# MasterBin-IIAU/Unicorn

Measured on AMD Instinct MI355X. Metric: frames/sec @ 800x1280 unicorn_track_large, higher is better.
Workload: dtype f16x2 (fp32-equivalent: split-f16 MFMA operands, fp32 accumulate); 1 GPU; unicorn_track_large SOT per-frame step 800x1280 (backbone+FPN, deform interaction, embedding, fp32-equivalent correlation, head); one independent stream per GPU, 16 consecutive frames per step; model=unicorn_track_large, task=sot, precision=f16x2, streams=1, distinct_frames_per_batch=16, weights=synthetic (oracle/synth.py), corr_dtype=f32-equivalent (f16x2 split operands, fp32 accumulate), accum=f32

## Files before the change

unicorn_amd/csrc/gemm_h2q.hip:

```cpp
#include "kernels.h"
#include "gemm_epi.h"


namespace {
constexpr int NW = 8;
constexpr int BM = 256, BN = 256, BKE = 32, ROWB = 128;
constexpr int HALF = 128 * ROWB;
constexpr int STAGE = 4 * HALF;
constexpr int OPER = 2 * STAGE;
constexpr int STG = 4096;
constexpr int LDS_BYTES = OPER + NW * STG;

struct Tile { int m0, n0, k0, split; };
struct ATile { __amdgpu_buffer_rsrc_t rs; int vo[2][2]; };
__device__ __forceinline__ Tile tile_of(int u, int nbm, int nbn, int nku) {
    const SplitTilePos t = supertile_split_pos(u, nbm, nbn, BM, BN);
    return {t.bm, t.bn, t.split * nku, t.split};
}
}

#define Q_WAIT_LDS() asm volatile("s_waitcnt lgkmcnt(0)" ::: "memory")

template <int ACT, bool OUTF, bool CONV, bool STATS, int FMT>
__global__ __launch_bounds__(64 * NW) void gemm_h2q_kernel(GemmArgs p) {
    constexpr int EB = FMT == FMT_H2 ? 4 : 2;
    constexpr int KS = ROWB / EB;
    extern __shared__ __attribute__((aligned(16))) char smem[];
    const int tid = threadIdx.x;
    const int lane = tid & 63;
    const int wave = __builtin_amdgcn_readfirstlane(tid >> 6);
    const int grp = wave >> 2, wc = wave & 3;
    const int fr = lane & 31, fh = lane >> 5;

    const int nbm = (p.M + BM - 1) / BM, nbn = (p.N + BN - 1) / BN;
    const int nunits = nbm * nbn * (p.splitk > 1 ? p.splitk : 1);
    int first, stride, count;
    persistent_units(blockIdx.x, gridDim.x, nunits, first, stride, count);
    if (count == 0) return;

    const int lrow = lane >> 3;
    const int lch = (lane & 7) ^ ((4 * (wave & 1) + (lrow >> 1)) & 7);
    const int lda4 = p.lda * EB, ldw4 = p.Kpad * EB;
    int vob[2][2];
#pragma unroll
    for (int h = 0; h < 2; ++h)
#pragma unroll
        for (int i = 0; i < 2; ++i) vob[h][i] = ((wave >> 2) * 64 + 8 * (wave & 3) + lrow + 128 * i + 32 * h) * ldw4 + lch * 16;
    const int arow = 8 * wave + lrow;
    auto make_a = [&](Tile tl, ATile& c) __attribute__((always_inline)) {
        char* abase = const_cast<char*>(reinterpret_cast<const char*>(p.A));
        if (!CONV) {
            const int rows = min(BM, p.M - tl.m0);
            c.rs = __builtin_amdgcn_make_buffer_rsrc(abase + (long)tl.m0 * lda4, 0, rows * lda4, 0x00020000);
#pragma unroll
            for (int h = 0; h < 2; ++h)
#pragma unroll
                for (int i = 0; i < 2; ++i) c.vo[h][i] = (arow + 128 * i + 64 * h) * lda4 + lch * 16;
        } else {
            const int b0 = tl.m0 / p.Mper, q0 = tl.m0 - b0 * p.Mper, oy0 = q0 / p.Wout, ox0 = q0 - oy0 * p.Wout;
            const int pix0 = (b0 * p.Hin + oy0 * p.stride) * p.Win + ox0 * p.stride;
            c.rs = __builtin_amdgcn_make_buffer_rsrc(abase + ((long)pix0 - (p.pad * p.Win + p.pad)) * lda4, 0, 0x7ffffff0, 0x00020000);
#pragma unroll
            for (int h = 0; h < 2; ++h)
#pragma unroll
                for (int i = 0; i < 2; ++i) {
                    const int m = tl.m0 + arow + 128 * i + 64 * h;
                    const bool ok = m < p.M;
                    const int mm = ok ? m : tl.m0;
                    const int b = mm / p.Mper, q = mm - b * p.Mper, oy = q / p.Wout, ox = q - oy * p.Wout;
                    const int off = ((b * p.Hin + oy * p.stride) * p.Win + ox * p.stride - pix0) * lda4 + lch * 16;
                    int bits = 0;
#pragma unroll
                    for (int t = 0; t < 3; ++t) {
                        const int iy = oy * p.stride - p.pad + t, ix = ox * p.stride - p.pad + t;
                        bits |= (t < p.KH && iy >= 0 && iy < p.Hin) ? (1 << t) : 0;
                        bits |= (t < p.KW && ix >= 0 && ix < p.Win) ? (8 << t) : 0;
                    }
                    c.vo[h][i] = off | ((ok ? bits : 0) << 26);
                }
        }
    };
    auto rsrc_b = [&](Tile tl) __attribute__((always_inline)) {
        return __builtin_amdgcn_make_buffer_rsrc(const_cast<char*>(reinterpret_cast<const char*>(p.W)) + (long)tl.n0 * ldw4, 0, BN * ldw4, 0x00020000);
    };
    const int cs = CONV ? p.Cin / KS : 1;
    const int csm = tap_csm(cs);
    const int kwm = tap_kwm(p.KW);
    auto issueA = [&](int h, int par, int kt, const ATile& c) __attribute__((always_inline)) {
        char* dst = smem + par * STAGE + h * HALF + wave * 1024;
        if (!CONV) {
            lds_dma16_buf(c.rs, dst, c.vo[h][0], kt * ROWB);
            lds_dma16_buf(c.rs, dst + 8192, c.vo[h][1], kt * ROWB);
        } else {
            const int tap = tap_index(kt, csm), cstep = kt - tap * cs;
            const int ky = tap_row(tap, kwm), kx = tap - ky * p.KW;
            const int soff = (ky * p.Win + kx) * lda4 + cstep * ROWB;
#pragma unroll
            for (int i = 0; i < 2; ++i) {
                const bool ok = ((c.vo[h][i] >> (26 + ky)) & (c.vo[h][i] >> (29 + kx)) & 1) != 0;
                lds_dma16_buf(c.rs, dst + i * 8192, ok ? (c.vo[h][i] & DESC_OFFSET_MASK) : DESC_OUT_OF_RANGE, soff);
            }
        }
    };
    auto issueB = [&](int h, int par, int kt, __amdgpu_buffer_rsrc_t rs) __attribute__((always_inline)) {
        char* dst = smem + par * STAGE + (2 + h) * HALF + wave * 1024;
        lds_dma16_buf(rs, dst, vob[h][0], kt * ROWB);
        lds_dma16_buf(rs, dst + 8192, vob[h][1], kt * ROWB);
    };

    const int sw = (fr >> 1) & 7;
    const int q0 = FMT == FMT_H2 ? 2 * fh : fh, q1 = FMT == FMT_H2 ? 2 * fh + 1 : 2 + fh;
    const int q2 = FMT == FMT_H2 ? 4 + 2 * fh : 4 + fh, q3 = FMT == FMT_H2 ? 5 + 2 * fh : 6 + fh;
    const int a_rd = (grp * 64 + fr) * ROWB, b_rd = 2 * HALF + (wc * 32 + fr) * ROWB;
    const int lds0 = (int)(size_t)(__attribute__((address_space(3))) char*)smem;
    if (lds0 != 0) __builtin_trap();
    int ra4[4] = {lds0 + a_rd + ((q0 ^ sw) << 4), lds0 + a_rd + ((q1 ^ sw) << 4), lds0 + a_rd + ((q2 ^ sw) << 4), lds0 + a_rd + ((q3 ^ sw) << 4)};
    int rb4[4] = {lds0 + b_rd + ((q0 ^ sw) << 4), lds0 + b_rd + ((q1 ^ sw) << 4), lds0 + b_rd + ((q2 ^ sw) << 4), lds0 + b_rd + ((q3 ^ sw) << 4)};

    f32x16 acc[4][2];
    f16x8 fa[2][4], fb[2][4];
    const int nk = (p.K / KS) / (p.splitk > 1 ? p.splitk : 1);
    Tile cur = tile_of(first, nbm, nbn, nk);
    Tile nxt = count > 1 ? tile_of(first + stride, nbm, nbn, nk) : cur;
    ATile ta_cur, ta_nxt;
    make_a(cur, ta_cur);
    make_a(nxt, ta_nxt);
    __amdgpu_buffer_rsrc_t rb_cur = rsrc_b(cur), rb_nxt = rsrc_b(nxt);

#define Q_LD_A(h)                                                                                   \
    _Pragma("unroll") for (int i = 0; i < 2; ++i) _Pragma("unroll") for (int q = 0; q < 4; ++q)      \
        fa[i][q] = lds_read_f16x8(ra4[q] + (h) * HALF + i * 32 * ROWB);
#define Q_LD_B(h) _Pragma("unroll") for (int q = 0; q < 4; ++q) fb[h][q] = lds_read_f16x8(rb4[q] + (h) * HALF);
#define Q_MF16(b, a, c) c = __builtin_amdgcn_mfma_f32_32x32x16_f16(b, a, c, 0, 0, 0)
#define Q_MB16(b, a, c) c = __builtin_amdgcn_mfma_f32_32x32x16_bf16(__builtin_bit_cast(bf16x8, b), __builtin_bit_cast(bf16x8, a), c, 0, 0, 0)
#define Q_MFMA(HA, HB)                                                                                   \
    if (FMT == FMT_H2) {                                                                                 \
        _Pragma("unroll") for (int kk = 0; kk < 2; ++kk) {                                               \
            Q_MF16(fb[HB][2 * kk + 1], fa[0][2 * kk], acc[2 * (HA)][HB]);                                \
            Q_MF16(fb[HB][2 * kk + 1], fa[1][2 * kk], acc[2 * (HA) + 1][HB]);                            \
            Q_MF16(fb[HB][2 * kk], fa[0][2 * kk + 1], acc[2 * (HA)][HB]);                                \
            Q_MF16(fb[HB][2 * kk], fa[1][2 * kk + 1], acc[2 * (HA) + 1][HB]);                            \
            Q_MF16(fb[HB][2 * kk], fa[0][2 * kk], acc[2 * (HA)][HB]);                                    \
            Q_MF16(fb[HB][2 * kk], fa[1][2 * kk], acc[2 * (HA) + 1][HB]);                                \
        }                                                                                                \
    } else {                                                                                             \
        _Pragma("unroll") for (int kk = 0; kk < 4; ++kk) {                                               \
            Q_MB16(fb[HB][kk], fa[0][kk], acc[2 * (HA)][HB]);                                            \
            Q_MB16(fb[HB][kk], fa[1][kk], acc[2 * (HA) + 1][HB]);                                        \
        }                                                                                                \
    }
#define Q_FUT(ahead)                                                   \
    int fk = kt + (ahead);                                             \
    const bool fnx = fk >= nk;                                         \
    fk -= fnx ? nk : 0;                                                \
    fk += fnx ? nxt.k0 : cur.k0;               \
    const __amdgpu_buffer_rsrc_t fb = fnx ? rb_nxt : rb_cur;                                  \
    ATile fa;                                                                                  \
    fa.rs = fnx ? ta_nxt.rs : ta_cur.rs;                                                       \
    _Pragma("unroll") for (int h_ = 0; h_ < 2; ++h_) _Pragma("unroll") for (int i_ = 0; i_ < 2; ++i_) {  \
        fa.vo[h_][i_] = (CONV && fnx) ? ta_nxt.vo[h_][i_] : ta_cur.vo[h_][i_];                 \
    }

    {
        const int kt = 0;
        issueA(0, 0, cur.k0, ta_cur); issueB(0, 0, cur.k0, rb_cur); issueB(1, 0, cur.k0, rb_cur); issueA(1, 0, cur.k0, ta_cur);
        Q_FUT(1);
        issueA(0, 1, fk, fa); issueB(1, 1, fk, fb); issueA(1, 1, fk, fa);
    }
    wait_vmcnt<6>();
    phase_barrier();
    if (grp == 1) phase_barrier();
    int par = 0;
#pragma unroll 1
    for (int t = 0; t < count; ++t) {
        ACC_CLEAR(acc, 4, 2);
#pragma unroll 1
        for (int kt = 0; kt < nk; ++kt) {
            {
                Q_LD_A(0); Q_LD_B(0);
                Q_WAIT_LDS();
                phase_barrier();
                if (!(p.dbg & 2)) { Q_MFMA(0, 0); }
                phase_barrier();
            }
            {
                Q_LD_B(1);
                if (!(p.dbg & 1)) { Q_FUT(1); issueB(0, par ^ 1, fk, fb); }
                if (!(p.dbg & 1)) { Q_FUT(2); issueA(0, par, fk, fa); }
                Q_WAIT_LDS();
                phase_barrier();
                if (!(p.dbg & 2)) { Q_MFMA(0, 1); }
                phase_barrier();
            }
            {
                Q_LD_A(1);
                Q_WAIT_LDS();
                phase_barrier();
                if (!(p.dbg & 2)) { Q_MFMA(1, 1); }
                phase_barrier();
            }
            {
                if (!(p.dbg & 1)) { Q_FUT(2); issueB(1, par, fk, fb); issueA(1, par, fk, fa); }
                wait_vmcnt<6>();
                Q_WAIT_LDS();
                phase_barrier();
                if (!(p.dbg & 2)) { Q_MFMA(1, 0); }
                phase_barrier();
            }
            par ^= 1;
#pragma unroll
            for (int q = 0; q < 4; ++q) { ra4[q] ^= STAGE; rb4[q] ^= STAGE; }
        }
        const Tile done = cur;
        cur = nxt; ta_cur = ta_nxt; rb_cur = rb_nxt;
        if (t + 2 < count) { nxt = tile_of(first + (t + 2) * stride, nbm, nbn, nk); make_a(nxt, ta_nxt); rb_nxt = rsrc_b(nxt); }
        char* st = smem + OPER + wave * STG;
        const int nw0 = done.n0 + wc * 64;
        const int rb0 = done.m0 + grp * 128;
        const int srow = p.splitk > 1 ? done.split * p.M : 0;
        if (p.dbg & 16) {
            float sacc = 0.f;
#pragma unroll
            for (int i = 0; i < 4; ++i)
#pragma unroll
                for (int j = 0; j < 2; ++j)
#pragma unroll
                    for (int r = 0; r < 16; ++r) sacc += acc[i][j][r];
            if (sacc == 1.2345e-30f && p.outF) p.outF[0] = sacc;
            continue;
        }
        if (STATS) {
            if (grp == 0) phase_barrier();
#pragma unroll
            for (int i = 0; i < 4; ++i)
#pragma unroll
                for (int j = 0; j < 2; ++j)
#pragma unroll
                    for (int r = 0; r < 16; ++r) acc[i][j][r] *= p.wscale;
        }
        const float ws = STATS ? 1.f : p.wscale;
        const bool has_res = OUTF && !STATS && !CONV && p.res != nullptr, has_b = p.outB != nullptr;
#pragma unroll
        for (int j = 0; j < 2; ++j) {
            float bv[16];
            {
                typedef float f32x8 __attribute__((ext_vector_type(8)));
                const __attribute__((address_space(4))) float* bias = (const __attribute__((address_space(4))) float*)(p.bias);
                if (!p.bias) {
#pragma unroll
                    for (int r = 0; r < 16; ++r) bv[r] = 0.f;
                } else if (nw0 + 64 <= p.N) {
#pragma unroll
                    for (int g = 0; g < 4; ++g) {
                        const f32x8 b8 = *reinterpret_cast<const __attribute__((address_space(4))) f32x8*>(bias + nw0 + j * 32 + 8 * g);
#pragma unroll
                        for (int e = 0; e < 4; ++e) bv[4 * g + e] = fh ? b8[4 + e] : b8[e];
                    }
                } else {
#pragma unroll
                    for (int g = 0; g < 4; ++g)
#pragma unroll
                        for (int e = 0; e < 4; ++e) {
                            const int c = nw0 + j * 32 + 8 * g + e;
                            const float lo = bias[min(c, p.N - 1)], hi = bias[min(c + 4, p.N - 1)];
                            bv[4 * g + e] = fh ? hi : lo;
                        }
                }
            }
#pragma unroll
            for (int i = 0; i < 4; ++i) {
                f32x4 rv[4];
                if (has_res) {
                    const int c = lane & 7, rr = lane >> 3;
                    const int col = nw0 + j * 32 + 4 * c;
#pragma unroll
                    for (int tt = 0; tt < 4; ++tt) {
                        const int row = rb0 + i * 32 + tt * 8 + rr;
                        const bool ok = row < p.M && col < p.N;
                        rv[tt] = *reinterpret_cast<const f32x4*>(p.res + (ok ? (size_t)row * p.ldr + col : 0));
                    }
                }
#pragma unroll
                for (int g = 0; g < 4; ++g) {
                    f32x4 v;
#pragma unroll
                    for (int e = 0; e < 4; ++e) v[e] = act_fast<ACT>(fmaf(acc[i][j][4 * g + e], ws, bv[4 * g + e]));
                    *reinterpret_cast<f32x4*>(st + fr * 128 + (((2 * g + fh) ^ (fr & 7)) << 4)) = v;
                }
                wave_lds_fence();
                if (OUTF) {
                    const int c = lane & 7, rr = lane >> 3;
                    const int col = nw0 + j * 32 + 4 * c;
#pragma unroll
                    for (int tt = 0; tt < 4; ++tt) {
                        const int r = tt * 8 + rr, row = rb0 + i * 32 + r;
                        f32x4 v = *reinterpret_cast<const f32x4*>(st + r * 128 + ((c ^ (r & 7)) << 4));
                        if (has_res) v += rv[tt];
                        if (row < p.M && col < p.N && !(p.dbg & 4)) {
                            const int orow = (p.out_hw ? (row / p.out_hw) * p.out_stride + p.out_off + row % p.out_hw : row) + srow;
                            *reinterpret_cast<f32x4*>(p.outF + (size_t)orow * p.ldf + col) = v;
                            if (has_b) act_store4(p.outB, (size_t)row * p.ldb + col, v[0], v[1], v[2], v[3], FMT);
                        }
                    }
                } else {
                    const int c = lane & 3, rr = lane >> 2;
                    const int col = nw0 + j * 32 + 8 * c;
#pragma unroll
                    for (int tt = 0; tt < 2; ++tt) {
                        const int r = tt * 16 + rr, row = rb0 + i * 32 + r;
                        const f32x4 lo = *reinterpret_cast<const f32x4*>(st + r * 128 + (((2 * c) ^ (r & 7)) << 4));
                        const f32x4 hi = *reinterpret_cast<const f32x4*>(st + r * 128 + (((2 * c + 1) ^ (r & 7)) << 4));
                        if (row < p.M && col < p.N && !(p.dbg & 4)) {
                            const float v8[8] = {lo[0], lo[1], lo[2], lo[3], hi[0], hi[1], hi[2], hi[3]};
                            if (FMT == FMT_H2) {
                                f16x8 h, l;
#pragma unroll
                                for (int q = 0; q < 8; ++q) { f16 hh, ll; h2_split(v8[q], hh, ll); h[q] = hh; l[q] = ll; }
                                char* op = reinterpret_cast<char*>(p.outB) + ((size_t)row * p.ldb + col) * 4;
                                __builtin_nontemporal_store(__builtin_bit_cast(f32x4, h), reinterpret_cast<f32x4*>(op));
                                __builtin_nontemporal_store(__builtin_bit_cast(f32x4, l), reinterpret_cast<f32x4*>(op + 16));
                            } else {
                                bf16x8 o;
#pragma unroll
                                for (int q = 0; q < 8; ++q) o[q] = (bf16)v8[q];
                                __builtin_nontemporal_store(__builtin_bit_cast(f32x4, o), reinterpret_cast<f32x4*>(p.outB + (size_t)row * p.ldb + col));
                            }
                        }
                    }
                }
                wave_lds_fence();
            }
        }
        if (STATS) {
            gemm_stats<2, 4, 4, 2>(p, acc, done.m0, done.n0, grp, wc, lane, tid, reinterpret_cast<float*>(smem + OPER));
            __syncthreads();
            if (grp == 1) phase_barrier();
        }
    }
    wait_vmcnt<0>();
    if (grp == 0) phase_barrier();
}

template <int ACT, bool OUTF, bool CONV, bool STATS, int FMT>
static int launch_h2q_inst(const GemmArgs& a, int grid, hipStream_t s) {
    static DevOnce attr_once;
    UNI_LDS_OPTIN(attr_once, "gemm_h2q", LDS_BYTES, reinterpret_cast<const void*>(&gemm_h2q_kernel<ACT, OUTF, CONV, STATS, FMT>));
    uni_note_gemm(OUTF ? "h2q_outF" : "h2q_outB", 188, CONV, STATS, a);
    hipLaunchKernelGGL((gemm_h2q_kernel<ACT, OUTF, CONV, STATS, FMT>), dim3(grid), dim3(64 * NW), LDS_BYTES, s, a);
    return 0;
}

bool gemm_h2q_supported(const GemmArgs& a) {
    const bool conv = gemm_is_conv(a);
    if (a.b32 != FMT_H2 && a.b32 != FMT_BF16) return false;
    const int ks = a.b32 == FMT_H2 ? 32 : 64, eb = a.b32 == FMT_H2 ? 4 : 2;
    if (!a.epi || a.K % ks != 0 || a.K < 2 * ks || a.act_col0 != 0) return false;
    if (!conv && !a.stats) {
        if (a.b32 != FMT_H2) return gemm_p44_supported(a);
        return a.out_hw == 0 && (a.act == ACT_NONE || a.act == ACT_RELU || a.act == ACT_GELU) && (a.outF || a.outB) && (a.outF || !a.res);
    }
    if (conv) {
        if (a.Cin % ks != 0 || a.KH > 3 || a.KW > 3 || a.K != a.KH * a.KW * a.Cin || a.Cin / ks > TAP_DECODE_MAX_CS) return false;
        const long span_pix = ((long)BM / a.Wout + 2) * a.stride * a.Win + (long)BM * a.stride + 3L * a.Win;
        if (span_pix * a.lda * eb >= (1L << 26)) return false;
    }
    if (a.res) return false;
    if (a.stats) return a.act == ACT_NONE && a.outF != nullptr && a.cpg > 0 && 256 / a.cpg + 2 <= 64;
    return a.outF != nullptr ? (a.act == ACT_NONE || a.act == ACT_RELU) : (a.outB != nullptr && !a.res && !a.out_hw && (a.act == ACT_NONE || a.act == ACT_RELU));
}

template <int FMT>
static int launch_h2q_fmt(const GemmArgs& a, int grid, hipStream_t s) {
    const bool f = a.outF != nullptr;
    const bool conv = gemm_is_conv(a);
    if (a.stats) return conv ? launch_h2q_inst<ACT_NONE, true, true, true, FMT>(a, grid, s) : launch_h2q_inst<ACT_NONE, true, false, true, FMT>(a, grid, s);
    if (conv) {
        if (a.act == ACT_RELU) return f ? launch_h2q_inst<ACT_RELU, true, true, false, FMT>(a, grid, s) : launch_h2q_inst<ACT_RELU, false, true, false, FMT>(a, grid, s);
        return f ? launch_h2q_inst<ACT_NONE, true, true, false, FMT>(a, grid, s) : launch_h2q_inst<ACT_NONE, false, true, false, FMT>(a, grid, s);
    }
    switch (a.act) {
        case ACT_GELU: return f ? launch_h2q_inst<ACT_GELU, true, false, false, FMT>(a, grid, s) : launch_h2q_inst<ACT_GELU, false, false, false, FMT>(a, grid, s);
        case ACT_RELU: return f ? launch_h2q_inst<ACT_RELU, true, false, false, FMT>(a, grid, s) : launch_h2q_inst<ACT_RELU, false, false, false, FMT>(a, grid, s);
        default: return f ? launch_h2q_inst<ACT_NONE, true, false, false, FMT>(a, grid, s) : launch_h2q_inst<ACT_NONE, false, false, false, FMT>(a, grid, s);
    }
}

int launch_gemm_h2q(const GemmArgs& a, hipStream_t s) {
    static int ncu = 0;
    if (!ncu) {
        const int n = uni_device_cus();
        if (!n) return -1;
        ncu = n - n % 8;
    }
    const int sk = a.splitk > 1 ? a.splitk : 1;
    const int ntiles = cdiv(a.M, BM) * cdiv(a.N, BN) * sk;
    const int grid = ntiles < ncu ? (ntiles + 7) / 8 * 8 : ncu;
    if (sk > 1) {
        GemmArgs g = gemm_splitk_partial_args(a);
        int rc = launch_h2q_fmt<FMT_H2>(g, grid, s);
        return rc ? rc : launch_splitk_reduce(a, s);
    }
    return a.b32 == FMT_H2 ? launch_h2q_fmt<FMT_H2>(a, grid, s) : launch_h2q_fmt<FMT_BF16>(a, grid, s);
}
```

Baseline: 160.5 frames/s.

## Hoist next-tile B prefetch before epilogue and use buffer-descriptor stores

Issues the first B-operand prefetch for the next tile before the epilogue runs, so global loads overlap with epilogue stores. The first-k-step wait count is widened to cover the outstanding epilogue stores. For the H2 format, the epilogue writes through a bounds-checked buffer resource instead of per-row branches, and residual loads are double-buffered one block ahead. This adds vmcnt bookkeeping complexity and relies on buffer out-of-range clamping for edge tiles.

Result: no change. 162.0 frames/s (median of 6 runs) (+0.9%).

```diff
diff --git a/unicorn_amd/csrc/gemm_h2q.hip b/unicorn_amd/csrc/gemm_h2q.hip
--- a/unicorn_amd/csrc/gemm_h2q.hip
+++ b/unicorn_amd/csrc/gemm_h2q.hip
@@ -1,5 +1,6 @@
 #include "kernels.h"
 #include "gemm_epi.h"
+#include <type_traits>
 
 
 namespace {
@@ -9,6 +10,7 @@
 constexpr int STAGE = 4 * HALF;
 constexpr int OPER = 2 * STAGE;
 constexpr int STG = 4096;
+constexpr int AUX_NT = 2;
 constexpr int LDS_BYTES = OPER + NW * STG;
 
 struct Tile { int m0, n0, k0, split; };
@@ -171,6 +173,10 @@
     phase_barrier();
     if (grp == 1) phase_barrier();
     int par = 0;
+    constexpr int EPI_VM = STATS ? 0 : (OUTF || FMT == FMT_H2) ? 32 : 16;
+    constexpr bool HOIST = !OUTF;
+    bool b0_ahead = false;
+    int epi_vm = 0;
 #pragma unroll 1
     for (int t = 0; t < count; ++t) {
         ACC_CLEAR(acc, 4, 2);
@@ -185,7 +191,7 @@
             }
             {
                 Q_LD_B(1);
-                if (!(p.dbg & 1)) { Q_FUT(1); issueB(0, par ^ 1, fk, fb); }
+                if (!(p.dbg & 1) && !(HOIST && b0_ahead)) { Q_FUT(1); issueB(0, par ^ 1, fk, fb); }
                 if (!(p.dbg & 1)) { Q_FUT(2); issueA(0, par, fk, fa); }
                 Q_WAIT_LDS();
                 phase_barrier();
@@ -201,7 +207,11 @@
             }
             {
                 if (!(p.dbg & 1)) { Q_FUT(2); issueB(1, par, fk, fb); issueA(1, par, fk, fa); }
-                wait_vmcnt<6>();
+                if (!HOIST || epi_vm == 0) wait_vmcnt<6>();
+                else if (epi_vm == 1) wait_vmcnt<6 + EPI_VM>();
+                else wait_vmcnt<(6 + 2 * EPI_VM < 63 ? 6 + 2 * EPI_VM : 63)>();
+                b0_ahead = false;
+                epi_vm = 0;
                 Q_WAIT_LDS();
                 phase_barrier();
                 if (!(p.dbg & 2)) { Q_MFMA(1, 0); }
@@ -214,6 +224,10 @@
         const Tile done = cur;
         cur = nxt; ta_cur = ta_nxt; rb_cur = rb_nxt;
         if (t + 2 < count) { nxt = tile_of(first + (t + 2) * stride, nbm, nbn, nk); make_a(nxt, ta_nxt); rb_nxt = rsrc_b(nxt); }
+        if (HOIST && !(p.dbg & 1)) { const int kt = 0; Q_FUT(1); issueB(0, par ^ 1, fk, fb); }
+        b0_ahead = HOIST;
+        asm volatile("" ::: "memory");
+        __builtin_amdgcn_sched_barrier(0);
         char* st = smem + OPER + wave * STG;
         const int nw0 = done.n0 + wc * 64;
         const int rb0 = done.m0 + grp * 128;
@@ -239,7 +253,46 @@
                     for (int r = 0; r < 16; ++r) acc[i][j][r] *= p.wscale;
         }
         const float ws = STATS ? 1.f : p.wscale;
-        const bool has_res = OUTF && !STATS && !CONV && p.res != nullptr, has_b = p.outB != nullptr;
+        const bool has_b = p.outB != nullptr;
+        unsigned all_lanes = ~0u;
+        asm volatile("" : "+s"(all_lanes));
+        const int elane = __builtin_amdgcn_mbcnt_hi(all_lanes, __builtin_amdgcn_mbcnt_lo(all_lanes, 0));
+        const int efr = elane & 31, efh = elane >> 5;
+        constexpr bool DESC = !CONV && !STATS && FMT == FMT_H2;
+        __amdgpu_buffer_rsrc_t rs_o;
+        int vo_o[2];
+        if (DESC) {
+            const int rows_w = min(128, p.M - rb0), cols_w = min(64, p.N - nw0);
+            const bool any = rows_w > 0 && cols_w > 0 && !(p.dbg & 4);
+            const int ld = OUTF ? p.ldf : p.ldb;
+            char* base = OUTF ? reinterpret_cast<char*>(p.outF + ((size_t)(rb0 + srow) * p.ldf + nw0))
+                              : reinterpret_cast<char*>(p.outB) + ((size_t)rb0 * p.ldb + nw0) * 4;
+            rs_o = __builtin_amdgcn_make_buffer_rsrc(base, 0, any ? ((rows_w - 1) * ld + cols_w) * 4 : 0, 0x00020000);
+#pragma unroll
+            for (int j = 0; j < 2; ++j) {
+                const int cl = j * 32 + (OUTF ? 4 * (elane & 7) : 8 * (elane & 3)), rr = OUTF ? elane >> 3 : elane >> 2;
+                vo_o[j] = nw0 + cl < p.N ? (rr * ld + cl) * 4 : DESC_OUT_OF_RANGE;
+            }
+            epi_vm = HOIST ? 1 : 0;
+        } else if (HOIST && !STATS && rb0 + 128 <= p.M && nw0 + 64 <= p.N && !(p.dbg & 4)) {
+            epi_vm = 1;
+        }
+        auto vo_of = [&](int j, int rb) __attribute__((always_inline)) { return (int)((unsigned)vo_o[j] + (unsigned)(rb * (OUTF ? p.ldf : p.ldb) * 4)); };
+        auto epilogue = [&](auto HR) __attribute__((always_inline)) {
+        constexpr bool has_res = decltype(HR)::value;
+        if (has_res && epi_vm) epi_vm = 2;
+        f32x4 rv[2][4];
+        auto load_res = [&](int i, int j, f32x4 (&r4)[4]) __attribute__((always_inline)) {
+            const int c = elane & 7, rr = elane >> 3;
+            const int col = nw0 + j * 32 + 4 * c;
+#pragma unroll
+            for (int tt = 0; tt < 4; ++tt) {
+                const int row = rb0 + i * 32 + tt * 8 + rr;
+                const bool ok = row < p.M && col < p.N;
+                r4[tt] = *reinterpret_cast<const f32x4*>(p.res + (ok ? (size_t)row * p.ldr + col : 0));
+            }
+        };
+        if (has_res) load_res(0, 0, rv[0]);
 #pragma unroll
         for (int j = 0; j < 2; ++j) {
             float bv[16];
@@ -254,7 +307,7 @@
                     for (int g = 0; g < 4; ++g) {
                         const f32x8 b8 = *reinterpret_cast<const __attribute__((address_space(4))) f32x8*>(bias + nw0 + j * 32 + 8 * g);
 #pragma unroll
-                        for (int e = 0; e < 4; ++e) bv[4 * g + e] = fh ? b8[4 + e] : b8[e];
+                        for (int e = 0; e < 4; ++e) bv[4 * g + e] = efh ? b8[4 + e] : b8[e];
                     }
                 } else {
 #pragma unroll
@@ -263,54 +316,57 @@
                         for (int e = 0; e < 4; ++e) {
                             const int c = nw0 + j * 32 + 8 * g + e;
                             const float lo = bias[min(c, p.N - 1)], hi = bias[min(c + 4, p.N - 1)];
-                            bv[4 * g + e] = fh ? hi : lo;
+                            bv[4 * g + e] = efh ? hi : lo;
                         }
                 }
             }
 #pragma unroll
             for (int i = 0; i < 4; ++i) {
-                f32x4 rv[4];
-                if (has_res) {
-                    const int c = lane & 7, rr = lane >> 3;
-                    const int col = nw0 + j * 32 + 4 * c;
-#pragma unroll
-                    for (int tt = 0; tt < 4; ++tt) {
-                        const int row = rb0 + i * 32 + tt * 8 + rr;
-                        const bool ok = row < p.M && col < p.N;
-                        rv[tt] = *reinterpret_cast<const f32x4*>(p.res + (ok ? (size_t)row * p.ldr + col : 0));
-                    }
-                }
+                constexpr int NB = 8;
+                const int bk = 4 * j + i;
 #pragma unroll
                 for (int g = 0; g < 4; ++g) {
                     f32x4 v;
 #pragma unroll
                     for (int e = 0; e < 4; ++e) v[e] = act_fast<ACT>(fmaf(acc[i][j][4 * g + e], ws, bv[4 * g + e]));
-                    *reinterpret_cast<f32x4*>(st + fr * 128 + (((2 * g + fh) ^ (fr & 7)) << 4)) = v;
+                    *reinterpret_cast<f32x4*>(st + efr * 128 + (((2 * g + efh) ^ (efr & 7)) << 4)) = v;
                 }
                 wave_lds_fence();
+                if (has_res && bk + 1 < NB) load_res((bk + 1) & 3, (bk + 1) >> 2, rv[(bk + 1) & 1]);
                 if (OUTF) {
-                    const int c = lane & 7, rr = lane >> 3;
+                    const int c = elane & 7, rr = elane >> 3;
                     const int col = nw0 + j * 32 + 4 * c;
 #pragma unroll
                     for (int tt = 0; tt < 4; ++tt) {
                         const int r = tt * 8 + rr, row = rb0 + i * 32 + r;
                         f32x4 v = *reinterpret_cast<const f32x4*>(st + r * 128 + ((c ^ (r & 7)) << 4));
-                        if (has_res) v += rv[tt];
-                        if (row < p.M && col < p.N && !(p.dbg & 4)) {
+                        if (has_res) v += rv[bk & 1][tt];
+                        if (DESC) {
+                            __builtin_amdgcn_raw_buffer_store_b128(__builtin_bit_cast(u32x4, v), rs_o, vo_of(j, i * 32 + tt * 8), 0, 0);
+                            if (has_b && row < p.M && col < p.N && !(p.dbg & 4)) act_store4(p.outB, (size_t)row * p.ldb + col, v[0], v[1], v[2], v[3], FMT);
+                        } else if (row < p.M && col < p.N && !(p.dbg & 4)) {
                             const int orow = (p.out_hw ? (row / p.out_hw) * p.out_stride + p.out_off + row % p.out_hw : row) + srow;
                             *reinterpret_cast<f32x4*>(p.outF + (size_t)orow * p.ldf + col) = v;
                             if (has_b) act_store4(p.outB, (size_t)row * p.ldb + col, v[0], v[1], v[2], v[3], FMT);
                         }
                     }
                 } else {
-                    const int c = lane & 3, rr = lane >> 2;
+                    const int c = elane & 3, rr = elane >> 2;
                     const int col = nw0 + j * 32 + 8 * c;
 #pragma unroll
                     for (int tt = 0; tt < 2; ++tt) {
                         const int r = tt * 16 + rr, row = rb0 + i * 32 + r;
                         const f32x4 lo = *reinterpret_cast<const f32x4*>(st + r * 128 + (((2 * c) ^ (r & 7)) << 4));
                         const f32x4 hi = *reinterpret_cast<const f32x4*>(st + r * 128 + (((2 * c + 1) ^ (r & 7)) << 4));
-                        if (row < p.M && col < p.N && !(p.dbg & 4)) {
+                        if (DESC) {
+                            const float v8[8] = {lo[0], lo[1], lo[2], lo[3], hi[0], hi[1], hi[2], hi[3]};
+                            f16x8 h, l;
+#pragma unroll
+                            for (int q = 0; q < 8; ++q) { f16 hh, ll; h2_split(v8[q], hh, ll); h[q] = hh; l[q] = ll; }
+                            const int vo = vo_of(j, i * 32 + tt * 16);
+                            __builtin_amdgcn_raw_buffer_store_b128(__builtin_bit_cast(u32x4, h), rs_o, vo, 0, AUX_NT);
+                            __builtin_amdgcn_raw_buffer_store_b128(__builtin_bit_cast(u32x4, l), rs_o, vo + 16, 0, AUX_NT);
+                        } else if (row < p.M && col < p.N && !(p.dbg & 4)) {
                             const float v8[8] = {lo[0], lo[1], lo[2], lo[3], hi[0], hi[1], hi[2], hi[3]};
                             if (FMT == FMT_H2) {
                                 f16x8 h, l;
@@ -330,6 +386,13 @@
                 }
                 wave_lds_fence();
             }
+        }
+        };
+        if constexpr (OUTF && !STATS && !CONV) {
+            if (p.res != nullptr) epilogue(std::true_type{});
+            else epilogue(std::false_type{});
+        } else {
+            epilogue(std::false_type{});
         }
         if (STATS) {
             gemm_stats<2, 4, 4, 2>(p, acc, done.m0, done.n0, grp, wc, lane, tid, reinterpret_cast<float*>(smem + OPER));
```
